# zehreken/fo-rma

Hardware: AMD Instinct MI355X
Metric: Msamples/sec (pixels×spp) at 1920×1080, 256 spp, 8 bounces; 1/2/4/8 GPU (higher is better)
Workload: dtype f32

## Files before the change

fo-rma_amd/csrc/rt_core.h:

```cpp
#pragma once
#include <stdint.h>

#if defined(__HIPCC_RTC__)
#define FR_HD __host__ __device__ __forceinline__
#elif defined(__HIPCC__) || defined(__HIP__)
#include <hip/hip_runtime.h>
#define FR_HD __host__ __device__ __forceinline__
#else
#include <math.h>
#define FR_HD static inline
#endif

namespace fr {

struct V3 {
  float x, y, z;
};

FR_HD V3 mk(float x, float y, float z) { return V3{x, y, z}; }
FR_HD V3 add(V3 a, V3 b) { return V3{a.x + b.x, a.y + b.y, a.z + b.z}; }
FR_HD V3 sub(V3 a, V3 b) { return V3{a.x - b.x, a.y - b.y, a.z - b.z}; }
FR_HD V3 mul(V3 a, V3 b) { return V3{a.x * b.x, a.y * b.y, a.z * b.z}; }
FR_HD V3 scl(float s, V3 a) { return V3{s * a.x, s * a.y, s * a.z}; }
FR_HD V3 divs(V3 a, float s) { return V3{a.x / s, a.y / s, a.z / s}; }
// ... 306 lines not shown
  return s;
}

constexpr float kBoxInvClamp = 0x1p100f;
FR_HD float box_inv_clamp(float inv) { return fmin_num(fmax_num(inv, -kBoxInvClamp), kBoxInvClamp); }
FR_HD bool recip_box_ok(float x) {
  const float ax = __builtin_fabsf(x);
  return (ax >= 0x1p-100f) & (ax < 0x1p126f);
}
FR_HD float fmin3_abs(float a, float b, float c) {
#if defined(__HIP_DEVICE_COMPILE__)
  float r;
  asm("v_min3_f32 %0, |%1|, |%2|, |%3|" : "=v"(r) : "v"(a), "v"(b), "v"(c));
  return r;
#else
  return fminf(fminf(fabsf(a), fabsf(b)), fabsf(c));
#endif
}
FR_HD bool recip_box_ok3(V3 d) {
  const float sum = (__builtin_fabsf(d.x) + __builtin_fabsf(d.y)) + __builtin_fabsf(d.z);
  return (fmin3_abs(d.x, d.y, d.z) >= 0x1p-100f) & (sum < 0x1p126f);
}
#if defined(__HIP__)
__device__ __forceinline__ V3 seg_box_inv(V3 d) {
  V3 inv{recip_nr(d.x), recip_nr(d.y), recip_nr(d.z)};
  if (!recip_box_ok3(d)) {
    inv = V3{1.0f / d.x, 1.0f / d.y, 1.0f / d.z};
    inv = V3{box_inv_clamp(inv.x), box_inv_clamp(inv.y), box_inv_clamp(inv.z)};
  }
  return inv;
}
#endif
FR_HD Slab slab3_box(V3 lo, V3 hi, V3 o, V3 inv, V3 oinv) {
  (void)o;
  return slab3_fused(lo, hi, oinv, inv);
}

FR_HD bool slab_root(const Slab& s, float t_min, float t_max, float& t) {
  t = s.tn > t_min ? s.tn : s.tf;
  return (t > t_min) & (t < t_max) & (s.tn < s.tf);
}

FR_HD float comp(V3 v, int k) { return k == 0 ? v.x : (k == 1 ? v.y : v.z); }

FR_HD V3 axis_normal(int k, float s) {
  return V3{k == 0 ? s : 0.0f, k == 1 ? s : 0.0f, k == 2 ? s : 0.0f};
}

FR_HD V3 slab_normal(const Slab& s, float t, V3 dd) {
#if defined(__HIP_DEVICE_COMPILE__)
  const bool entry = t == s.tn;
  const float mnx = fmin_num(s.t0.x, s.t1.x), mxx = fmax_num(s.t0.x, s.t1.x);
  const float mny = fmin_num(s.t0.y, s.t1.y), mxy = fmax_num(s.t0.y, s.t1.y);
  const bool kx = (entry ? mnx : mxx) == t;
  const bool ky = !kx && (entry ? mny : mxy) == t;
  const bool kz = !kx && !ky;
  const float dk = kx ? dd.x : (ky ? dd.y : dd.z);
  const float sg = ((dk > 0.0f) != entry) ? 1.0f : -1.0f;
  return V3{kx ? sg : 0.0f, ky ? sg : 0.0f, kz ? sg : 0.0f};
#else
  if (t == s.tn) {
    const int k = fmin_num(s.t0.x, s.t1.x) == s.tn ? 0 : (fmin_num(s.t0.y, s.t1.y) == s.tn ? 1 : 2);
    return axis_normal(k, comp(dd, k) > 0.0f ? -1.0f : 1.0f);
  }
  const int k = fmax_num(s.t0.x, s.t1.x) == s.tf ? 0 : (fmax_num(s.t0.y, s.t1.y) == s.tf ? 1 : 2);
  return axis_normal(k, comp(dd, k) > 0.0f ? 1.0f : -1.0f);
#endif
}

FR_HD bool tri_root(V3 v0, V3 e1, V3 e2, V3 o, V3 d, float t_min, float t_max, float& t) {
  const V3 pv = cross(d, e2);
  const float inv_det = 1.0f / dot(e1, pv);
  const V3 s = sub(o, v0);
  const float u = dot(s, pv) * inv_det;
  const V3 qv = cross(s, e1);
  const float v = dot(d, qv) * inv_det;
  t = dot(e2, qv) * inv_det;
  return (u >= 0.0f) & (v >= 0.0f) & (u + v <= 1.0f) & (t > t_min) & (t < t_max);
}

struct ObbFrame {
  V3 dl, inv, ol;
};

FR_HD ObbFrame obb_frame(V3 c, V3 ax, V3 ay, V3 az, V3 o, V3 d) {
  ObbFrame f;
  const V3 oc = sub(o, c);
  f.ol = V3{dot(ax, oc), dot(ay, oc), dot(az, oc)};
  f.dl = V3{dot(ax, d), dot(ay, d), dot(az, d)};
  f.inv = V3{1.0f / f.dl.x, 1.0f / f.dl.y, 1.0f / f.dl.z};
  return f;
}

FR_HD V3 obb_normal(V3 ax, V3 ay, V3 az, const Slab& s, float t, V3 dl) {
  const V3 nl = slab_normal(s, t, dl);
  const float sg = nl.x + nl.y + nl.z;
  const V3 axis = nl.x != 0.0f ? ax : (nl.y != 0.0f ? ay : az);
  return scl(sg, axis);
}

enum ScatterClass : uint32_t { SC_LAMBERT = 0, SC_METAL = 1, SC_DIELECTRIC = 2, SC_LIGHT = 3, SC_NONE = 4 };

FR_HD V3 scatter_lambert(V3 p, V3 n, Rng& r) {
  const V3 target = add(add(p, n), random_in_unit_sphere(r));
  return sub(target, p);
}

FR_HD bool scatter_metal(V3 d, V3 p_unused, V3 n, float fuzz, Rng& r, V3& dir) {
  (void)p_unused;
  const V3 refl = reflect(unit(d), n);
  dir = add(refl, scl(fuzz, random_in_unit_sphere(r)));
  return dot(dir, n) > 0.0f;
}

FR_HD V3 scatter_dielectric(V3 d, V3 n, Rng& r) {
  const float ref_idx = 1.3f;
  const V3 reflected = reflect(d, n);
  V3 outward;
  float ni, cosine;
  const float dn = dot(d, n);
  if (dn > 0.0f) {
    outward = sub(V3{0.0f, 0.0f, 0.0f}, n);
    ni = ref_idx;
    cosine = ref_idx * dot(d, n) / length(d);
  } else {
    outward = n;
    ni = 1.0f / ref_idx;
    cosine = -dot(d, n) / length(d);
  }
  const V3 uv = unit(d);
  const float dt = dot(uv, outward);
  const float disc = 1.0f - ni * ni * (1.0f - dt * dt);
  V3 refracted = V3{0.0f, 0.0f, 0.0f};
  float reflect_prob;
  if (disc > 0.0f) {
    refracted = sub(scl(ni, sub(uv, scl(dt, outward))), scl(sqrtf(disc), outward));
    reflect_prob = schlick(cosine, ref_idx);
  } else {
    reflect_prob = 1.0f;
  }
  return rng_f32(r) < reflect_prob ? reflected : refracted;
}

FR_HD float sky_t(V3 d) {
  const V3 ud = unit(d);
  return 0.5f * (ud.y + 1.0f);
}
FR_HD float sky_t_from(float dy, float dd) { return 0.5f * (dy / sqrtf(dd) + 1.0f); }
FR_HD V3 sky_from_t(float t) { return add(scl(1.0f - t, V3{1.0f, 1.0f, 1.0f}), scl(t, V3{0.5f, 0.7f, 1.0f})); }
FR_HD V3 sky(V3 d) { return sky_from_t(sky_t(d)); }

#if defined(__HIP__)
__device__ __forceinline__ float sky_t_fast_from(float dy, float dd) {
  const bool fast = (dd >= 0x1p-96f) & (dd <= 0x1p126f);
  if (fast) {
#if defined(__HIP_DEVICE_COMPILE__)
    const float s = __builtin_amdgcn_sqrtf(dd);
    const float sdn = __uint_as_float(__float_as_uint(s) - 1u);
    const float sup = __uint_as_float(__float_as_uint(s) + 1u);
    const float rdn = __builtin_fmaf(-sdn, s, dd);
    const float rup = __builtin_fmaf(-sup, s, dd);
    float len = rdn <= 0.0f ? sdn : s;
    len = rup > 0.0f ? sup : len;
    const float q = div_rn(dy, len, recip_nr(len));
    return 0.5f * (q + 1.0f);
#endif
  }
  return sky_t_from(dy, dd);
}
__device__ __forceinline__ float sky_t_fast(V3 d) {
  return sky_t_fast_from(d.y, d.x * d.x + d.y * d.y + d.z * d.z);
}
#endif

FR_HD uint8_t to_u8(float c) {
  const float s = sqrtf(c) * 255.0f;
  if (!(s > 0.0f)) return 0;
  if (s >= 255.0f) return 255;
  return static_cast<uint8_t>(s);
}

FR_HD uint8_t as_u8_trunc(float v) {
  if (!(v > 0.0f)) return 0;
  if (v >= 255.0f) return 255;
  return static_cast<uint8_t>(v);
}

}
```

fo-rma_amd/csrc/trace_kernel.h:

```cpp
#pragma once
#if !defined(__HIPCC_RTC__)
#include <hip/hip_runtime.h>
#include <float.h>
#include <type_traits>
#include "../../include/forma_rt.h"
#include "bvh.h"
#else
#include <type_traits>
#include "forma_rt.h"
#include "bvh.h"
#ifndef FLT_MAX
#define FLT_MAX __FLT_MAX__
#endif
#endif

#ifdef FR_DIAG
__device__ unsigned long long g_fr_diag_lens[2];
__device__ unsigned long long g_fr_diag_rus[2];
#define FR_DIAG_TRY(arr)                                                           \
  do {                                                                             \
    const unsigned long long m_ = __ballot(1);                                     \
    if ((threadIdx.x & 63u) == static_cast<uint32_t>(__ffsll(m_) - 1)) {             \
      atomicAdd(&arr[0], 1ull);                                                    \
      atomicAdd(&arr[1], static_cast<unsigned long long>(__popcll(m_)));           \
// ... 159 lines not shown
    const unsigned long long m_ = __ballot(1);                                       \
    if ((k) < SC_N && lane == static_cast<uint32_t>(__ffsll(m_) - 1)) {            \
      atomicAdd(&sec_cnt[(k) < SC_N ? (k) : 0], 1u);                               \
      atomicAdd(&sec_cnt[SC_N + ((k) < SC_N ? (k) : 0)], lanes_in(m_));            \
    }                                                                                \
  } while (0)
#else
#define SEC(k) do {} while (0)
#endif

extern "C" __device__ bool fr_inverse_ballot(unsigned long long) __asm("llvm.amdgcn.inverse.ballot.i64");
__device__ __forceinline__ bool lane_in(unsigned long long m) { return fr_inverse_ballot(m); }

__device__ __forceinline__ uint32_t lanes_in(unsigned long long m) {
  return static_cast<uint32_t>(__builtin_popcount(static_cast<uint32_t>(m)) +
                               __builtin_popcount(static_cast<uint32_t>(m >> 32)));
}
__device__ __forceinline__ uint32_t lanes_in_once(unsigned long long m) {
  uint32_t c = static_cast<uint32_t>(__builtin_popcountll(m));
#if defined(__HIP_DEVICE_COMPILE__)
  asm("" : "+s"(c));
#endif
  return c;
}
__device__ __forceinline__ uint32_t lanes_set(bool b) { return lanes_in(__builtin_amdgcn_ballot_w64(b)); }

__device__ __forceinline__ uint32_t lds_addr(const uint32_t* p) {
  return static_cast<uint32_t>(reinterpret_cast<uintptr_t>((__attribute__((address_space(3))) const uint32_t*)p));
}
__device__ __forceinline__ __attribute__((address_space(3))) uint32_t& lds_u32_at(uint32_t a) {
  return *reinterpret_cast<__attribute__((address_space(3))) uint32_t*>(static_cast<uintptr_t>(a));
}
__device__ __forceinline__ uint32_t lane_sel(unsigned long long m, uint32_t if_set, uint32_t if_clear) {
#if defined(__HIP_DEVICE_COMPILE__)
  uint32_t r;
  asm("v_cndmask_b32 %0, %1, %2, %3" : "=v"(r) : "v"(if_clear), "v"(if_set), "s"(m));
  return r;
#else
  return if_set;
#endif
}

__device__ __forceinline__ uint32_t slot_tile(const KParams& kp, uint32_t q) {
  uint32_t tile = q >> 6;
#if defined(__HIP_DEVICE_COMPILE__)
  if (kp.flags & KF_LIST) tile = kp.tile_list[__builtin_amdgcn_readfirstlane(tile)];
#endif
  return tile;
}

template <bool LIST = true>
__device__ __forceinline__ bool slot_xy(const KParams& kp, uint32_t q, uint32_t& x, uint32_t& y) {
  const uint32_t tile = LIST ? slot_tile(kp, q) : q >> 6, l = q & 63u;
  const uint32_t ls = fastdiv(tile, kp.row_magic, kp.row_shift);
  const uint32_t tc = tile - ls * kp.tiles_per_row;
  const uint32_t strip = kp.shard_index + ls * kp.shard_count;
  x = tc * 8u + (l & 7u);
  y = strip * kStripRows + (l >> 3);
  return x < kp.W && y < kp.H;
}

__device__ __forceinline__ bool item_xy(const KParams& kp, uint32_t item, uint32_t& bw, uint32_t& q, uint32_t& x,
                                        uint32_t& y) {
  const bool fine = item >= kp.n_coarse;
  const uint32_t tb = (fine ? item - kp.n_coarse : item) >> 6;
  const uint32_t bl = fastdiv(tb, kp.tiles_magic, kp.tiles_shift);
  bw = fine ? (kp.b_fine | kFineKey | (bl << 28)) : kp.b0 + bl;
  q = ((tb - bl * kp.n_tiles) << 6) | (item & 63u);
  return slot_xy(kp, q, x, y);
}

__host__ __device__ __forceinline__ uint32_t stream_key(uint32_t bw) {
  return (bw & kFineKey) ? (kFineKey | ((bw & 0x0FFFFFFFu) * kFineSub + ((bw >> 28) & 3u))) : bw;
}

__device__ __forceinline__ BatchEntry batch_entry(const KParams& kp, uint32_t item) {
  uint32_t bw, q, x, y;
  const bool in_image = item_xy(kp, item, bw, q, x, y);
  const Rng st = rng_seed(kp.seed, y * kp.W + x, stream_key(bw));
  const uint32_t k = (bw >> 28) & 3u;
  const bool fine = (bw & kFineKey) != 0u;
  const uint32_t first = k * kFineSamples;
  const uint32_t left = kp.spp - (bw & 0x0FFFFFFFu) * kBlockSamples;
  const uint32_t span = first + (fine ? kFineSamples : kBlockSamples);
  const uint32_t end = span < left ? span : left;
  const bool ok = in_image && item < kp.n_items;
  BatchEntry e;
  e.s0 = st.s0;
  e.s1 = st.s1;
  e.s2 = st.s2;
  e.s3 = st.s3;
  e.fx = static_cast<float>(x) * 16777216.0f + 8388608.0f;
  e.fy = static_cast<float>(kp.H - y) * 16777216.0f + 8388608.0f;
  const uint64_t slot = static_cast<uint64_t>(item - k * kp.P) * kp.ks;
  e.se = (ok ? (first | (end << 8) | (kNeedJit << 16)) : 0u) | (static_cast<uint32_t>(slot >> 32) << 24);
  e.slot = static_cast<uint32_t>(slot);
  return e;
}

typedef uint32_t u32x4 __attribute__((ext_vector_type(4)));
__device__ __forceinline__ __attribute__((address_space(3))) u32x4& lds_u32x4_at(uint32_t a) {
  return *reinterpret_cast<__attribute__((address_space(3))) u32x4*>(static_cast<uintptr_t>(a));
}
__device__ __forceinline__ void wave_lds_order() {
#if defined(__HIP_DEVICE_COMPILE__)
  __builtin_amdgcn_fence(__ATOMIC_SEQ_CST, "wavefront");
  __builtin_amdgcn_wave_barrier();
#endif
}


template <uint32_t I, uint32_t N, class F>
__device__ __forceinline__ void unroll_below(uint32_t n, F& f) {
  if constexpr (I < N) {
    if (I < n) {
      f(std::integral_constant<uint32_t, I>{});
      unroll_below<I + 1u, N>(n, f);
    }
  }
}

#ifdef FR_JIT_N
constexpr uint32_t kJitRec[FR_JIT_N][16] = {FR_JIT_REC};
template <uint32_t I>
struct JitRec {
  __device__ __forceinline__ float4 operator[](int k) const {
    return make_float4(__builtin_bit_cast(float, kJitRec[I][4 * k]), __builtin_bit_cast(float, kJitRec[I][4 * k + 1]),
                       __builtin_bit_cast(float, kJitRec[I][4 * k + 2]),
                       __builtin_bit_cast(float, kJitRec[I][4 * k + 3]));
  }
};
#endif

template <int KS, bool HAS_PLANE, int KREJ, int MAXD, bool BVH, bool MT, int DEFER, int MAT = 0>
#define FR_OCC_ATTR                                                                                      \
  __attribute__((amdgpu_waves_per_eu(FR_MIN_WAVES ? FR_MIN_WAVES : BVH ? FR_BVH_WAVES                 \
                                                      : DEFER == 2 ? FR_NIB_WAVES                       \
                                                      : (DEFER == 1 && MAT == 1) ? FR_DIFF12_WAVES : 7)))
__global__ __launch_bounds__(kBlock) __attribute__((amdgpu_num_sgpr(FR_NUM_SGPR))) FR_OCC_ATTR void trace_kernel(
    KArgs args) {
  const KScene& sc = args.sc;
  const KParams& kp = args.kp;
  const KWork& kw = args.kw;
  extern __shared__ uint32_t lds[];
  constexpr bool NIB = DEFER == 2;
  constexpr uint32_t STG = stage_samples(BVH, NIB);
  constexpr bool DIFFUSE = MAT == 1;
  constexpr uint32_t WPS = NIB ? 2u : 3u;
  constexpr bool TABLE = has_batch_table(BVH, NIB);
  constexpr uint32_t TABW = TABLE ? kBatchTableBytes / 4u : 0u;
  static_assert(!TABLE || !MT, "a batch-table entry holds no render_mt band offset");
  const bool staged = STG > 1 && (!BVH || NIB || (kp.flags & KF_STAGE) != 0u);
  float* stage = reinterpret_cast<float*>(lds) + TABW + threadIdx.x * (WPS * STG);
  constexpr bool ATT_LDS = DEFER != 0 && !BVH, REC_LDS = NIB && !BVH;
  static_assert(kDeferMaxPrims <= kAttLds && kNibbleMaxPrims <= kRecLds, "LDS staging bounds");
  const uint32_t n_att = ATT_LDS || sc.n <= kAttLds ? sc.n : 0u;
  const uint32_t n_att_st = n_att ? n_att + 1u : 0u;
  const uint32_t n_rec = REC_LDS || sc.n <= kRecLds ? sc.n : 0u;
  float4* att_lds = reinterpret_cast<float4*>(lds + TABW + (staged ? kBlock * WPS * STG : 0u));
  float4* rec_lds = att_lds + n_att_st;
  uint32_t* stack = reinterpret_cast<uint32_t*>(rec_lds + 4u * n_rec);
  uint16_t* hstack = reinterpret_cast<uint16_t*>(stack);
  const uint32_t tid = threadIdx.x;
  const uint32_t lane = tid & 63u;
  static_assert(MAXD == 0 || MAXD == 8, "the u16 stack is one 16-B row per lane");
  static_assert(!DEFER || (MAXD == 8 && !MT && (!BVH || (NIB && DIFFUSE))),
                "deferred unwind: depth <= 8 list kernels, or diffuse BVH kernels with 8-B records");
  uint2* drow = reinterpret_cast<uint2*>(stack) + tid;
  uint8_t* bstack = reinterpret_cast<uint8_t*>(stack);
  uint4* hrow = reinterpret_cast<uint4*>(stack) + tid;
  uint32_t* tstack = stack + (NIB ? 0u : MAXD ? (MAXD * kBlock) / 2u : (kp.max_depth ? kp.max_depth : 1u) * kBlock);
  constexpr uint32_t kLevelB = 4u * kBlock;
  const uint32_t tbase = lds_addr(tstack) + kLevelB;
  if (BVH) tstack[tid] = kBvhEnd;
  const uint32_t ent_shift = n_att ? 4u : 0u;
  const uint32_t unit_ent = sc.n << ent_shift;
  const uint32_t unit2 = unit_ent | (unit_ent << 16);
  if (DEFER == 1)
    *drow = make_uint2(~0u, ~0u);
  else if (!DEFER && MAXD > 0)
    *hrow = make_uint4(unit2, unit2, unit2, unit2);
  for (uint32_t i = tid; i < n_att_st; i += kBlock) {
    const float4 a = sc.att[i];
    att_lds[i] = make_float4(a.x, a.y, a.z, __uint_as_float(i < n_att ? sc.cls[i] : 0u));
  }
  for (uint32_t i = tid; i < 4u * n_rec; i += kBlock) rec_lds[i] = sc.rec[i];
#ifdef FR_DIAG
  __shared__ uint32_t dg[DG_N];
  if (tid < DG_N) dg[tid] = 0;
  const uint32_t gw = blockIdx.x * (kBlock / 64u) + (tid >> 6);
  if (lane == 0 && gw < 65536) {
    g_fr_wave_times[2 * gw] = __builtin_amdgcn_s_memrealtime();
    g_fr_wave_drain[gw] = ~0ull;
  }
#endif
#ifdef FR_SECCNT
  __shared__ uint32_t sec_cnt[2 * SC_N];
  if (tid < 2 * SC_N) sec_cnt[tid] = 0;
#endif
  __syncthreads();


  enum : uint32_t { NEED_NONE = 0, NEED_LENS = 1, NEED_SPHERE = 2, NEED_JIT = 3 };
  static_assert(NEED_JIT == kNeedJit && NEED_NONE == 0u, "a batch-table entry holds the claim's need");
  uint32_t depth = 0;
  uint32_t wnib = ~0u;
  const uint32_t dmask = kp.max_depth ? (0xFu << (4u * (8u - min(kp.max_depth, 8u)))) : 0u;
  auto push = [&](uint32_t pi) {
    if (NIB)
      wnib = (wnib >> 4) | (pi << 28);
    else if (DEFER)
      bstack[tid * 8u + depth] = static_cast<uint8_t>(pi);
    else if (MAXD > 0)
      hstack[tid * MAXD + depth] = static_cast<uint16_t>(pi << ent_shift);
    else
      stack[depth * kBlock + tid] = pi;
  };

  V3 o{0.0f, 0.0f, 0.0f}, d{0.0f, 0.0f, 1.0f};
  V3 sn{0.0f, 0.0f, 0.0f};
  float sfuzz = 0.0f, fx = 0.0f, fy = 0.0f, vofs = 0.0f;
  bool smetal = false;
  uint32_t sbest = 0, s = 0, s_end = 0, nseg = 0, nhit = 0;
  static_assert((kBlockSamples & (kBlockSamples - 1u)) == 0u, "blocks of a power-of-two sample count");
#ifdef FR_DIAG
  uint32_t diag_tb = 0, diag_seg0 = 0;
  uint32_t diag_iter = 0;
#endif
  float* out = kw.samples;
  Rng rng{0u, 0u, 0u, 0u};
  bool active = true, have_ray = false;
  uint32_t need = NEED_NONE;

#ifdef FR_PROF
  uint64_t pf_acc[PF_N] = {0, 0, 0, 0, 0};
  uint64_t pf_t = __builtin_amdgcn_s_memtime();
#endif
  uint32_t q_next = 0, q_end = 0;
  Rng held{0u, 0u, 0u, 0u};
  uint32_t held_xy = 0xFFFFFFFFu, held_b = 0u;
  const uint32_t tab_mine = lds_addr(lds) + tid * kBatchEntryBytes;
  auto seed_entry = [&](const KParams& kq, uint32_t item) {
    const BatchEntry e = batch_entry(kq, item);
    lds_u32x4_at(tab_mine) = u32x4{e.s0, e.s1, e.s2, e.s3};
    lds_u32x4_at(tab_mine + 16u) = u32x4{__float_as_uint(e.fx), __float_as_uint(e.fy), e.se, e.slot};
  };
  {
    const KParams k0 = kernarg_reload(args, [](const auto& a) { return a.kp; });
    q_next = (blockIdx.x * (kBlock / 64u) + (tid >> 6)) * kBatch;
    q_end = q_next + kBatch;
    if constexpr (TABLE) {
      seed_entry(k0, q_next + lane);
      wave_lds_order();
    } else {
      uint32_t bb, qq, xx, yy;
      const bool in_image = item_xy(k0, q_next + lane, bb, qq, xx, yy);
      held = rng_seed(k0.seed, yy * k0.W + xx, stream_key(bb));
      held_xy = in_image ? (xx | (yy << 16)) : 0xFFFFFFFFu;
      held_b = bb;
    }
  }
  while (active) {
    SEC(SC_ITER);
    DIAG_WAVE(DG_ITER);
#ifdef FR_DIAG
    if (lane == 0 && (gw & 63u) == 0 && (gw >> 6) < 1024u && diag_iter < 1024u)
      g_fr_iter_times[(gw >> 6) * 1024u + diag_iter] = __builtin_amdgcn_s_memrealtime();
    ++diag_iter;
#endif
    const unsigned long long m = __builtin_amdgcn_ballot_w64(s == s_end);
    constexpr uint32_t CLAIM_MIN = NIB ? (BVH ? FR_CLAIM_MIN_BVH : FR_CLAIM_MIN_NIB) : FR_CLAIM_MIN;
    if (m && (CLAIM_MIN <= 1 || lanes_in_once(m) >= CLAIM_MIN || m == __ballot(1))) {
      SEC(SC_CLAIM);
      const uint32_t n = static_cast<uint32_t>(__popcll(m));
      const uint32_t r = __builtin_amdgcn_mbcnt_hi(static_cast<uint32_t>(m >> 32),
                                                   __builtin_amdgcn_mbcnt_lo(static_cast<uint32_t>(m), 0u));
      const uint32_t next = __builtin_amdgcn_readfirstlane(q_next);
      const uint32_t avail = __builtin_amdgcn_readfirstlane(q_end) - next;
      if constexpr (TABLE) {
        const bool grab = avail == 0u;
        unsigned long long mc = m;
        uint32_t take = n, start = next;
        if (!grab && n > avail) {
          mc = m & __builtin_amdgcn_ballot_w64(r < avail);
          take = avail;
        }
        if (grab) {
          SEC(SC_GRAB);
          wave_lds_order();
          const int first = __ffsll(static_cast<long long>(m)) - 1;
          uint32_t base = 0;
          if (static_cast<int>(lane) == first) base = atomicAdd(kw.queue, kBatch);
          base = __builtin_amdgcn_readlane(base, first);
          const KParams kg = kernarg_reload(args, [](const auto& a) { return a.kp; });
          base += kg.n_static;
          q_end = base + kBatch;
          seed_entry(kg, base + lane);
          wave_lds_order();
          start = base;
        }
        q_next = start + take;
        const uint32_t item = start + r;
        if (lane_in(mc) && item >= kp.n_items) {
#ifdef FR_DIAG
          if (gw < 65536) {
            const unsigned long long now = __builtin_amdgcn_s_memrealtime();
            if (now < g_fr_wave_drain[gw]) {
              g_fr_wave_drain[gw] = now;
              g_fr_wave_iters[2 * gw] = diag_iter;
            }
          }
#endif
          active = false;
          continue;
        }
        if (lane_in(mc)) {
          SEC(SC_SETUP);
          const uint32_t ea = lds_addr(lds) + (tid & ~63u) * kBatchEntryBytes + (item & (kBatch - 1u)) * kBatchEntryBytes;
          const u32x4 e0 = lds_u32x4_at(ea), e1 = lds_u32x4_at(ea + 16u);
          rng = Rng{e0.x, e0.y, e0.z, e0.w};
          fx = __uint_as_float(e1.x);
          fy = __uint_as_float(e1.y);
          s = e1.z & 0xFFu;
          s_end = (e1.z >> 8) & 0xFFu;
          need = (e1.z >> 16) & 0xFFu;
          uint64_t slot = (static_cast<uint64_t>(e1.z >> 24) << 32) | e1.w;
#if defined(__HIP_DEVICE_COMPILE__)
          asm volatile("" : "+v"(slot));
#endif
          out = kw.samples + WPS * slot;
#ifdef FR_DIAG
          if (s != s_end) {
            diag_tb = item >> 6;
            diag_seg0 = nseg;
          }
#endif
        }
      } else {
        uint32_t base = 0;
        const bool grab = n > avail;
        const int first = __ffsll(static_cast<long long>(m)) - 1;
        int sl = static_cast<int>(((next + r) & (kBatch - 1u)) << 2);
        Rng st{static_cast<uint32_t>(__builtin_amdgcn_ds_bpermute(sl, static_cast<int>(held.s0))),
               static_cast<uint32_t>(__builtin_amdgcn_ds_bpermute(sl, static_cast<int>(held.s1))),
               static_cast<uint32_t>(__builtin_amdgcn_ds_bpermute(sl, static_cast<int>(held.s2))),
               static_cast<uint32_t>(__builtin_amdgcn_ds_bpermute(sl, static_cast<int>(held.s3)))};
        uint32_t xy = static_cast<uint32_t>(__builtin_amdgcn_ds_bpermute(sl, static_cast<int>(held_xy)));
        uint32_t b = static_cast<uint32_t>(__builtin_amdgcn_ds_bpermute(sl, static_cast<int>(held_b)));
        if (grab) {
          SEC(SC_GRAB);
          if (static_cast<int>(lane) == first) base = atomicAdd(kw.queue, kBatch);
          base = __builtin_amdgcn_readlane(base, first);
          const KParams kg = kernarg_reload(args, [](const auto& a) { return a.kp; });
          base += kg.n_static;
          q_end = base + kBatch;
          uint32_t bb, qq, xx, yy;
          const bool in_image = item_xy(kg, base + lane, bb, qq, xx, yy);
          held = rng_seed(kg.seed, yy * kg.W + xx, stream_key(bb));
          held_xy = in_image ? (xx | (yy << 16)) : 0xFFFFFFFFu;
          held_b = bb;
          sl = static_cast<int>(((r - avail) & (kBatch - 1u)) << 2);
          const Rng st2{static_cast<uint32_t>(__builtin_amdgcn_ds_bpermute(sl, static_cast<int>(held.s0))),
                        static_cast<uint32_t>(__builtin_amdgcn_ds_bpermute(sl, static_cast<int>(held.s1))),
                        static_cast<uint32_t>(__builtin_amdgcn_ds_bpermute(sl, static_cast<int>(held.s2))),
                        static_cast<uint32_t>(__builtin_amdgcn_ds_bpermute(sl, static_cast<int>(held.s3)))};
          const uint32_t xy2 = static_cast<uint32_t>(__builtin_amdgcn_ds_bpermute(sl, static_cast<int>(held_xy)));
          const uint32_t b2 = static_cast<uint32_t>(__builtin_amdgcn_ds_bpermute(sl, static_cast<int>(held_b)));
          if (r >= avail) {
            st = st2;
            xy = xy2;
            b = b2;
          }
        }
        q_next = grab ? base + (n - avail) : next + n;
        const uint32_t item = r < avail ? next + r : base + (r - avail);
        if (lane_in(m) && item >= kp.n_items) {
#ifdef FR_DIAG
          if (gw < 65536) {
            const unsigned long long now = __builtin_amdgcn_s_memrealtime();
            if (now < g_fr_wave_drain[gw]) {
              g_fr_wave_drain[gw] = now;
              g_fr_wave_iters[2 * gw] = diag_iter;
            }
          }
#endif
          active = false;
          continue;
        }
        if (lane_in(m)) {
          SEC(SC_SETUP);
          const uint32_t x = xy & 0xFFFFu, y = xy >> 16;
          bool ok = xy != 0xFFFFFFFFu;
          uint32_t yrow = kp.H - y;
          if (MT) {
            const uint32_t k = kp.band_h ? y / kp.band_h : 4u;
            ok = ok && k < 4u;
            yrow = kp.band_h - (y - k * kp.band_h);
            vofs = static_cast<float>(3u - k) * 0.25f;
          }
          if (ok) {
            rng = st;
            const uint32_t k = (b >> 28) & 3u;
            const bool fine = (b & kFineKey) != 0u;
            const uint32_t j0 = k * kFineSamples;
            s = (b & 0x0FFFFFFFu) * kBlockSamples + j0;
            out = kw.samples + WPS * (static_cast<size_t>(item - k * kp.P) * kp.ks);
#ifdef FR_DIAG
            diag_tb = item >> 6;
            diag_seg0 = nseg;
#endif
            s_end = min(s + (fine ? kFineSamples : kBlockSamples), kp.spp);
            fx = static_cast<float>(x) * 16777216.0f + 8388608.0f;
            fy = static_cast<float>(yrow) * 16777216.0f + 8388608.0f;
            need = NEED_JIT;
          }
        }
      }
    }
    PROF_MARK(PF_CLAIM);
    bool ended = false;
    V3 term{0.0f, 0.0f, 0.0f};
    uint32_t tsky;
#if defined(__HIP_DEVICE_COMPILE__)
    asm volatile("" : "=v"(tsky));
#else
    tsky = kDeferAbsorbed;
#endif
    if (need != NEED_NONE) {
      SEC(SC_NEED);
      const unsigned long long msph = __builtin_amdgcn_ballot_w64(need == NEED_SPHERE);
      float pz = 0.0f;
      DIAG_WAVE(DG_LENS_W);
      DIAG_LANE(DG_LENS_L);
      float px = rng_signed_unit_scaled(rng);
      float py = rng_signed_unit_scaled(rng);
      const unsigned long long mjit = __builtin_amdgcn_ballot_w64(need == NEED_JIT);
      float pw = 0.0f;
      if (lane_in(msph | mjit)) pw = rng_signed_unit_scaled(rng);
      if (lane_in(msph)) pz = pw;
      if (lane_in(mjit)) {
        SEC(SC_JIT);
        d.x = div_rn(fx + px, kp.sW, kp.rW);
        d.y = div_rn(fy + py, kp.sH, kp.rH);
        if (MT) d.y = d.y + vofs;
        px = pw;
        py = rng_signed_unit_scaled(rng);
        need = NEED_LENS;
      }
      float dd = px * px + py * py + pz * pz;
      unsigned long long mrej = __builtin_amdgcn_ballot_w64(dd >= kUnitBallScaled);
      while (lanes_in(mrej) > static_cast<uint32_t>(KREJ)) {
        SEC(SC_REJ);
        DIAG_WAVE(DG_LENS_W);
        DIAG_LANE(DG_LENS_L);
        if (lane_in(mrej)) {
          px = rng_signed_unit_scaled(rng);
          py = rng_signed_unit_scaled(rng);
          if (lane_in(msph)) pz = rng_signed_unit_scaled(rng);
          dd = px * px + py * py + pz * pz;
        }
        mrej = __builtin_amdgcn_ballot_w64(dd >= kUnitBallScaled);
      }
      SEC(SC_ACC);
      const unsigned long long macc = ~mrej;
      if (lane_in(macc & ~msph)) {
        SEC(SC_CAM);
        KCam cm = kernarg_reload(args, [](const auto& a) { return a.cam; });
#if defined(__HIP_DEVICE_COMPILE__)
        asm volatile("" : "+s"(cm.dz));
#endif
        const CamLens rd = cam_lens(cm, px, py);
        uint32_t general = (cm.lens_pre & kCamAxial) ^ kCamAxial;
#if defined(__HIP_DEVICE_COMPILE__)
        asm volatile("" : "+s"(general));
#endif
        if (cm.lens_pre & kCamAxial) {
          const CamRay cr = cam_ray_axial(cm, rd, d.x, d.y);
          o = cr.o;
          d = cr.d;
        }
        if (general) {
          const CamRay cr = cam_ray(cm, rd, d.x, d.y);
          o = cr.o;
          d = cr.d;
        }
        if (!NIB) depth = 0;
        have_ray = true;
      }
      if (lane_in(macc & msph)) {
        SEC(SC_SCAT);
        bool ok = true;
        V3 dir;
        if (!DIFFUSE && smetal) {
          const V3 r{px * kSignedUnitScale, py * kSignedUnitScale, pz * kSignedUnitScale};
          dir = add(d, scl(sfuzz, r));
          ok = dot(dir, sn) > 0.0f;
        } else {
          const V3 dr{__builtin_fmaf(px, kSignedUnitScale, d.x), __builtin_fmaf(py, kSignedUnitScale, d.y),
                      __builtin_fmaf(pz, kSignedUnitScale, d.z)};
          dir = sub(dr, o);
        }
        if (ok) {
          if (!(NIB && DIFFUSE)) push(sbest);
          if (!NIB) ++depth;
          d = dir;
          have_ray = true;
        } else {
          ended = true;
          tsky = kDeferAbsorbed;
        }
      }
      if (lane_in(macc)) need = NEED_NONE;
    }
    PROF_MARK(PF_REJ);
    if (have_ray) {
      SEC(SC_HIT);
      ++nseg;
      const V3 inv = seg_box_inv(d);
      const V3 boinv{o.x * inv.x, o.y * inv.y, o.z * inv.z};
      const float a_dd = dot(d, d);
      const SphereSeg ssg = sphere_seg(a_dd);
      float closest = FLT_MAX, t_last = 0.0f;
      int best = -1;
      bool list_walk = !BVH;
      if (BVH) {
        const float ao = fmax3_num(__builtin_fabsf(o.x), __builtin_fabsf(o.y), __builtin_fabsf(o.z));
        const float ad = fmax3_num(__builtin_fabsf(d.x), __builtin_fabsf(d.y), __builtin_fabsf(d.z));
        const float aoi = fmax3_num(__builtin_fabsf(boinv.x), __builtin_fabsf(boinv.y), __builtin_fabsf(boinv.z));
        list_walk = __ballot(!(ao <= sc.reach) | !(ad >= kBvhTinyDir) | !(aoi <= FLT_MAX)) != 0;
      }
      if (BVH && !list_walk) {
        typedef __attribute__((address_space(4))) const uint32_t cu32;
        for (uint32_t sg = 0; sg < sc.n_segs; ++sg) {
          const cu32* sp = (cu32*)(reinterpret_cast<uintptr_t>(sc.segs)) + 4u * __builtin_amdgcn_readfirstlane(sg);
          if (HAS_PLANE && sp[0]) {
            const uint32_t i = sp[3];
            const RecRef r4 = rec_at(sc.rec, i);
            float t = 0.0f;
            const int r = plane_test(xyz(r4[0]), xyz(r4[1]), xyz(r4[2]), o, d, 0.001f, closest, t);
            if (r) t_last = t;
            if (r == 2) {
              closest = t;
              best = static_cast<int>(i);
            }
            continue;
          }
          uint32_t ref = sp[1];
          uint32_t tso = tbase + 4u * tid;
          const V3 invc{__builtin_amdgcn_fmed3f(inv.x, -kBvhInvClamp, kBvhInvClamp),
                        __builtin_amdgcn_fmed3f(inv.y, -kBvhInvClamp, kBvhInvClamp),
                        __builtin_amdgcn_fmed3f(inv.z, -kBvhInvClamp, kBvhInvClamp)};
          const V3 oinv{o.x * invc.x, o.y * invc.y, o.z * invc.z};
          while (ref != kBvhEnd) {
            while (ref < kBvhLeaf) {
              SEC(SC_NODE);
              DIAG_WAVE(DG_NODE_W);
              DIAG_LANE(DG_NODE_L);
#ifdef FR_DIAG
              {
                unsigned long long m_ = __ballot(1);
                uint32_t u_ = 0;
                while (m_ && u_ < 5) {
                  const uint32_t r_ = __builtin_amdgcn_readlane(ref, __ffsll(m_) - 1);
                  m_ &= ~__ballot(ref == r_);
                  ++u_;
                }
                if (u_ == 1) DIAG_WAVE(DG_NCOH_W);
                if (u_ == 2) DIAG_WAVE(DG_NU2_W);
                if (u_ == 3 || u_ == 4) DIAG_WAVE(DG_NU4_W);
                if (depth == 0) DIAG_LANE(DG_NPRIM_L);
              }
#endif
              typedef unsigned long long Mask;
              const uint32_t tdown = tso - kLevelB;
              const uint32_t top = lds_u32_at(tdown);
              uint32_t t_near, t_far;
              Mask t_many, t_both;
              auto node_pick = [&](const Slab& sl, const Slab& sr, const uint32_t cl, const uint32_t cr) {
                const Mask ml = __builtin_amdgcn_ballot_w64(sl.tn <= sl.tf) &
                                __builtin_amdgcn_ballot_w64(sl.tf >= 0.001f) & __builtin_amdgcn_ballot_w64(sl.tn <= closest);
                const Mask mr = __builtin_amdgcn_ballot_w64(sr.tn <= sr.tf) &
                                __builtin_amdgcn_ballot_w64(sr.tf >= 0.001f) & __builtin_amdgcn_ballot_w64(sr.tn <= closest);
                const Mask mgol = ml & (__builtin_amdgcn_ballot_w64(sl.tn <= sr.tn) | ~mr);
                const Mask many = ml | mr;
                const uint32_t cx = cl ^ cr;
                const uint32_t near = cl ^ lane_sel(mgol, 0u, cx);
                t_near = near;
                t_far = near ^ cx;
                t_many = many;
                t_both = ml & mr;
              };
              auto node_step = [&](const float4 na, const float4 nb, const float4 nc, const uint32_t cl,
                                   const uint32_t cr) {
                node_pick(slab3_fused(xyz(na), xyz(nb), oinv, invc),
                          slab3_fused(V3{na.w, nc.x, nc.y}, V3{nb.w, nc.z, nc.w}, oinv, invc), cl, cr);
              };
              const uint32_t ref0 = __builtin_amdgcn_readfirstlane(ref);
              if (__ballot(ref != ref0) == 0) {
                const RecRef nd = rec_at(sc.bvh, ref0);
                const float4 r = nd[3];
                SEC(SC_NODES);
                node_step(nd[0], nd[1], nd[2], __float_as_uint(r.x), __float_as_uint(r.y));
                asm volatile("; bvh node step: scalar");
              } else {
                SEC(SC_NODEV);
                const uint32_t nb0 = ref * 64u;
                const uint4 nr = __builtin_bit_cast(uint4, buf_load4(sc.bvh, nb0 + 48u));
                node_step(buf_load4(sc.bvh, nb0), buf_load4(sc.bvh, nb0 + 16u), buf_load4(sc.bvh, nb0 + 32u), nr.x, nr.y);
                asm volatile("; bvh node step: vector");
              }
              SEC(SC_NODET);
              lds_u32_at(tso) = t_far;
              const uint32_t tpop = lane_sel(t_many, tso, tdown);
              ref = lane_sel(t_many, t_near, top);
              tso = lane_sel(t_both, tso + kLevelB, tpop);
            }
            if (ref == kBvhEnd) break;
            SEC(SC_LEAF);
            DIAG_WAVE(DG_LEAF_W);
            DIAG_LANE(DG_LEAF_L);
            auto leaf_test = [&](const uint32_t i, const auto& r) {
              const float tmax =
// ... 11 lines not shown
              } else if (k == FR_AABB) {
                h = slab_root(slab3_box(xyz(r[0]), xyz(r[1]), o, inv, boinv), 0.001f, tmax, t);
              } else if (k == FR_TRIANGLE) {
                h = tri_root(xyz(r[0]), xyz(r[1]), xyz(r[2]), o, d, 0.001f, tmax, t);
              } else if (k == FR_OBB) {
                const float4 a = r[0], b = r[1], c = r[2], e = r[3];
                const ObbFrame f = obb_frame(xyz(a), xyz(b), xyz(c), xyz(e), o, d);
                h = slab_root(slab3(V3{-a.w, -b.w, -c.w}, V3{a.w, b.w, c.w}, f.ol, f.inv), 0.001f, tmax, t);
              }
              if (h) {
                closest = t;
                best = static_cast<int>(i);
                if (HAS_PLANE) t_last = t;
              }
            };
            const uint32_t first = ref & ((1u << kBvhSlotBits) - 1u);
            const uint32_t cnt = ((ref >> kBvhSlotBits) & 15u) + 1u;
            const uint32_t leaf0 = __builtin_amdgcn_readfirstlane(ref);
            if (__ballot(ref != leaf0) == 0) {
              typedef __attribute__((address_space(4))) const uint32_t cu32l;
              const cu32l* ord = (cu32l*)(reinterpret_cast<uintptr_t>(sc.bvh_order));
              const uint32_t first0 = leaf0 & ((1u << kBvhSlotBits) - 1u);
              const uint32_t cnt0 = ((leaf0 >> kBvhSlotBits) & 15u) + 1u;
              for (uint32_t kk = 0; kk < cnt0; ++kk) {
                SEC(SC_LTESTS);
                leaf_test(ord[first0 + kk], rec_at(sc.lrec, first0 + kk));
              }
              asm volatile("; bvh leaf: scalar");
            } else {
              for (uint32_t kk = 0; kk < cnt; ++kk) {
                SEC(SC_LTESTV);
                const uint32_t slot = first + kk;
                struct LeafRec {
                  const float4* base;
                  uint32_t off;
                  __device__ float4 operator[](uint32_t k) const { return buf_load4(base, off + 16u * k); }
                } const r{sc.lrec, slot * 64u};
                leaf_test(buf_load1(sc.bvh_order, slot * 4u), r);
              }
              asm volatile("; bvh leaf: vector");
            }
            tso -= kLevelB;
            ref = lds_u32_at(tso);
          }
        }
      }
      auto test_rec = [&](auto kind_tag, uint32_t i, const auto& r4) {
        constexpr uint32_t K = decltype(kind_tag)::value;
        float t = 0.0f;
        bool h = false;
        if constexpr (K == FR_AABB) {
          h = slab_root(slab3_box(xyz(r4[0]), xyz(r4[1]), o, inv, boinv), 0.001f, closest, t);
        } else if constexpr (K == FR_SPHERE) {
          const float4 g = r4[0];
          h = sphere_root_fast(xyz(g), g.w, o, d, a_dd, ssg, 0.001f, closest, t);
        } else if constexpr (K == FR_PLANE) {
          const int r = plane_test(xyz(r4[0]), xyz(r4[1]), xyz(r4[2]), o, d, 0.001f, closest, t);
          if (r) t_last = t;
          h = r == 2;
        } else if constexpr (K == FR_TRIANGLE) {
          h = tri_root(xyz(r4[0]), xyz(r4[1]), xyz(r4[2]), o, d, 0.001f, closest, t);
        } else if constexpr (K == FR_OBB) {
          const float4 a = r4[0], b = r4[1], c = r4[2], e = r4[3];
          const ObbFrame f = obb_frame(xyz(a), xyz(b), xyz(c), xyz(e), o, d);
          h = slab_root(slab3(V3{-a.w, -b.w, -c.w}, V3{a.w, b.w, c.w}, f.ol, f.inv), 0.001f, closest, t);
        }
        if (h) {
          closest = t;
          best = static_cast<int>(i);
          if (HAS_PLANE) t_last = t;
        }
#if defined(FR_JIT_N) && defined(__HIP_DEVICE_COMPILE__)
        if constexpr (!std::is_same<typename std::decay<decltype(r4)>::type, RecRef>::value) {
          asm volatile("" : "+v"(best));
          if (HAS_PLANE) asm volatile("" : "+v"(t_last));
        }
#endif
      };
      auto test_one = [&](auto kind_tag, uint32_t i) {
        SEC(SC_LIST);
        test_rec(kind_tag, i, rec_at(sc.rec, i));
      };
      typedef std::integral_constant<uint32_t, FR_AABB> TagAabb;
      typedef std::integral_constant<uint32_t, FR_SPHERE> TagSphere;
#ifdef FR_JIT_N
      if constexpr (!BVH) {
        auto test_j = [&](auto ic) {
          constexpr uint32_t I = decltype(ic)::value;
          constexpr uint32_t K = kJitRec[I][15];
          if constexpr (K == FR_AABB || K == FR_SPHERE || K == FR_PLANE || K == FR_TRIANGLE || K == FR_OBB) {
            test_rec(std::integral_constant<uint32_t, K>{}, I, JitRec<I>{});
          }
        };
        unroll_below<0u, FR_JIT_N>(FR_JIT_N, test_j);
      } else
#endif
      if constexpr (NIB && !BVH && KS != KS_ANY) {
        auto test_k = [&](auto ic) {
          if constexpr (KS == KS_AABB)
            test_one(TagAabb{}, decltype(ic)::value);
          else
            test_one(TagSphere{}, decltype(ic)::value);
        };
        uint32_t n_here = sc.n;
#if defined(__HIP_DEVICE_COMPILE__)
        asm volatile("" : "+s"(n_here));
#endif
        unroll_below<0u, kNibbleMaxPrims>(n_here, test_k);
      } else if constexpr (KS != KS_ANY) {
        for (uint32_t ii = 0; ii < (list_walk ? sc.n : 0u); ++ii) {
          const uint32_t i = __builtin_amdgcn_readfirstlane(ii);
          if constexpr (KS == KS_AABB)
            test_one(TagAabb{}, i);
          else
            test_one(TagSphere{}, i);
        }
      } else {
        typedef __attribute__((address_space(4))) const uint32_t cu32r;
        for (uint32_t rr = 0; rr < (list_walk ? sc.n_runs : 0u); ++rr) {
          const cu32r* rp = (cu32r*)(reinterpret_cast<uintptr_t>(sc.runs)) + 4u * __builtin_amdgcn_readfirstlane(rr);
          const uint32_t k = rp[0], i0 = rp[1], i1 = rp[2];
          if (k == FR_AABB) {
            for (uint32_t i = i0; i < i1; ++i) test_one(TagAabb{}, __builtin_amdgcn_readfirstlane(i));
          } else if (k == FR_SPHERE) {
            for (uint32_t i = i0; i < i1; ++i) test_one(TagSphere{}, __builtin_amdgcn_readfirstlane(i));
          } else if (k == FR_PLANE) {
            for (uint32_t i = i0; i < i1; ++i)
              test_one(std::integral_constant<uint32_t, FR_PLANE>{}, __builtin_amdgcn_readfirstlane(i));
          } else if (k == FR_TRIANGLE) {
            for (uint32_t i = i0; i < i1; ++i)
              test_one(std::integral_constant<uint32_t, FR_TRIANGLE>{}, __builtin_amdgcn_readfirstlane(i));
          } else if (k == FR_OBB) {
            for (uint32_t i = i0; i < i1; ++i)
              test_one(std::integral_constant<uint32_t, FR_OBB>{}, __builtin_amdgcn_readfirstlane(i));
          }
        }
      }
      PROF_MARK(PF_HIT);
      SEC(SC_POSTHIT);
      if (best < 0) {
        SEC(SC_SKY);
        if (DEFER)
          tsky = __float_as_uint(sky_t_fast(d));
        else
          term = sky(d);
        ended = true;
        have_ray = false;
      } else {
        DIAG_WAVE(DG_HIT_W);
        ++nhit;
        ended = true;
        tsky = kDeferAbsorbed;
        have_ray = false;
        if (NIB ? (dmask != 0u && (wnib & dmask) == dmask) : depth < kp.max_depth) {
          SEC(SC_SHADE);
          const V3 pw = add(o, scl(closest, d));
          float4 b0, b1, b2, b3;
          if (REC_LDS || n_rec) {
            const float4* rb = rec_lds + 4 * best;
            b0 = rb[0];
            b1 = rb[1];
            b2 = rb[2];
            b3 = rb[3];
          } else {
            const uint32_t off = 64u * static_cast<uint32_t>(best);
            b0 = buf_load4(sc.rec, off);
            b1 = buf_load4(sc.rec, off + 16u);
            b2 = buf_load4(sc.rec, off + 32u);
            b3 = buf_load4(sc.rec, off + 48u);
          }
          const uint32_t c = (DIFFUSE && KS != KS_ANY) ? static_cast<uint32_t>(SC_LAMBERT)
                             : ATT_LDS || n_att        ? __float_as_uint(att_lds[best].w)
                                                       : buf_load1(sc.cls, 4u * best);
          const uint32_t kb = KS == KS_AABB ? FR_AABB : KS == KS_SPHERE ? FR_SPHERE : __float_as_uint(b3.w);
          V3 n;
          if (kb == FR_AABB) {
            n = slab_normal(slab3_box(xyz(b0), xyz(b1), o, inv, boinv), closest, d);
          } else if (kb == FR_SPHERE) {
            n = divs(sub(pw, xyz(b0)), b0.w);
          } else if (kb == FR_PLANE) {
            n = scl(-1.0f, xyz(b1));
          } else if (kb == FR_TRIANGLE) {
            n = xyz(b3);
            if (c != SC_DIELECTRIC && dot(n, d) > 0.0f) n = scl(-1.0f, n);
          } else {
            const ObbFrame f = obb_frame(xyz(b0), xyz(b1), xyz(b2), xyz(b3), o, d);
            const Slab sl = slab3(V3{-b0.w, -b1.w, -b2.w}, V3{b0.w, b1.w, b2.w}, f.ol, f.inv);
            n = obb_normal(xyz(b1), xyz(b2), xyz(b3), sl, closest, f.dl);
          }
          const V3 p = HAS_PLANE ? add(o, scl(t_last, d)) : pw;
          const V3 din = d;
          o = p;
          d = add(p, n);
          sbest = static_cast<uint32_t>(best);
          smetal = !DIFFUSE && c == SC_METAL;
          ended = c == SC_NONE;
          if (c != SC_NONE && (DIFFUSE || c != SC_DIELECTRIC)) need = NEED_SPHERE;
          if (NIB && DIFFUSE && c != SC_NONE) {
            if (BVH)
              push(buf_load1(sc.acls, 4u * static_cast<uint32_t>(best)));
            else
              push(static_cast<uint32_t>(best));
          }
          if (!DIFFUSE && c == SC_DIELECTRIC) {
            d = scatter_dielectric(din, n, rng);
            push(static_cast<uint32_t>(best));
            if (!NIB) ++depth;
            have_ray = true;
          } else if (smetal) {
            sfuzz = sc.mat[best].w;
            sn = n;
            d = reflect(unit(din), n);
          }
        }
      }
    }
    PROF_MARK(PF_SHADE);
    SEC(SC_POSTSHADE);
    if (ended) {
      SEC(SC_END);
      DIAG_WAVE(DG_END_W);
      DIAG_LANE(DG_END_L);
      V3 col = term;
      if (NIB) {
        col = V3{__uint_as_float(tsky), __uint_as_float(wnib), 0.0f};
        wnib = ~0u;
      } else if (DEFER) {
        const uint2 w = *drow;
        *drow = make_uint2(~0u, ~0u);
        col = V3{__uint_as_float(tsky), __uint_as_float(w.x), __uint_as_float(w.y)};
      } else if (MAXD > 0) {
        const uint4 w = *hrow;
        *hrow = make_uint4(unit2, unit2, unit2, unit2);
        const uint32_t ws[4] = {w.x, w.y, w.z, w.w};
        if (n_att) {
          const char* att_bytes = reinterpret_cast<const char*>(att_lds);
#pragma unroll
          for (int j = MAXD - 1; j >= 0; --j) {
            DIAG_WAVE(DG_UNW_W);
            const uint32_t off = (j & 1) ? (ws[j >> 1] >> 16) : (ws[j >> 1] & 0xFFFFu);
            col = mul(xyz(*reinterpret_cast<const float4*>(att_bytes + off)), col);
          }
        } else {
#pragma unroll
          for (int j = MAXD - 1; j >= 0; --j)
            if (j < static_cast<int>(depth)) col = mul(xyz(sc.att[(ws[j >> 1] >> (16 * (j & 1))) & 0xFFFFu]), col);
        }
      } else {
        const bool zero_term = (__float_as_uint(term.x) | __float_as_uint(term.y) | __float_as_uint(term.z)) == 0u;
        const int udepth = sc.att_nonneg && zero_term ? 0 : static_cast<int>(depth);
        if (n_att) {
          for (int j = udepth - 1; j >= 0; --j) {
            const uint32_t pi = stack[j * kBlock + tid];
            col = mul(xyz(att_lds[pi]), col);
          }
        } else {
          for (int j = udepth - 1; j >= 0; --j) col = mul(xyz(sc.att[stack[j * kBlock + tid]]), col);
        }
      }
      const uint32_t jj = s & (kBlockSamples - 1u);
      if (!staged) {
        out[WPS * jj] = col.x;
        out[WPS * jj + 1] = col.y;
        if (WPS == 3) out[WPS * jj + 2] = col.z;
      } else {
        float* sl = stage + WPS * (jj & (STG - 1u));
        sl[0] = col.x;
        sl[1] = col.y;
        if (WPS == 3) sl[2] = col.z;
        const bool full = (jj & (STG - 1u)) == STG - 1u;
        if (full || s + 1u == s_end) {
          float* dst = out + WPS * (jj & ~(STG - 1u));
          if (full && kp.ks == kBlockSamples) {
            if constexpr ((WPS * STG) % 4u == 0u) {
              const float4* src = reinterpret_cast<const float4*>(stage);
#pragma unroll
              for (uint32_t k = 0; k < WPS * STG / 4u; ++k) {
                reinterpret_cast<float4*>(dst)[k] = src[k];
#if defined(__HIP_DEVICE_COMPILE__)
                if (WPS * STG > 8u) asm volatile("" ::: "memory");
#endif
              }
            } else {
              const float2* src = reinterpret_cast<const float2*>(stage);
#pragma unroll
              for (uint32_t k = 0; k < WPS * STG / 2u; ++k) reinterpret_cast<float2*>(dst)[k] = src[k];
            }
          } else {
            for (uint32_t k = 0; k < WPS * ((jj & (STG - 1u)) + 1u); ++k) dst[k] = stage[k];
          }
        }
      }
#ifdef FR_DIAG
      if (s + 1u == s_end && diag_tb < (1u << 20)) atomicAdd(&g_fr_tb_cost[diag_tb], nseg - diag_seg0);
#endif
      if (++s != s_end) need = NEED_JIT;
    }
    PROF_MARK(PF_END);
    SEC(SC_LATCH);
  }

  unsigned long long a = nseg, b = nhit, sct = 0;
  for (int m = 32; m > 0; m >>= 1) {
    a += __shfl_xor(a, m);
    b += __shfl_xor(b, m);
    sct += __shfl_xor(sct, m);
  }
  if (lane == 0) {
    unsigned long long* wc = kw.wave_counters + 3u * (blockIdx.x * (kBlock / 64u) + (tid >> 6));
    wc[0] = a;
    wc[1] = b;
    wc[2] = sct;
  }
#ifdef FR_SECCNT
  __syncthreads();
  if (tid < SC_N) atomicAdd(&kw.counters[4 + tid], static_cast<unsigned long long>(sec_cnt[tid]));
  if (tid < SC_N) atomicAdd(&kw.counters[32 + tid], static_cast<unsigned long long>(sec_cnt[SC_N + tid]));
#endif
#ifdef FR_PROF
  if (lane == 0)
    for (int k = 0; k < PF_N; ++k) atomicAdd(&kw.counters[20 + k], static_cast<unsigned long long>(pf_acc[k]));
#endif
#ifdef FR_DIAG
  if (lane == 0 && gw < 65536) {
    g_fr_wave_times[2 * gw + 1] = __builtin_amdgcn_s_memrealtime();
    g_fr_wave_iters[2 * gw + 1] = diag_iter;
  }
  __syncthreads();
  if (tid < DG_N) atomicAdd(&kw.counters[4 + tid], static_cast<unsigned long long>(dg[tid]));
#endif
}

}
```

Measured before the change: 40000.

## Make trace loop control wave-uniform with live mask and scalar-friendly branching

Replaces the per-lane active flag with a wave-level live lane mask so the persistent loop exits uniformly, and turns per-lane claim/retire and staging-flush conditions into ballot masks. It also makes the sky-t fast path branchless, forces some values into scalar registers, rewrites the rejection loop as if/do-while, swaps shfl_xor for direct ds_bpermute, and adds an optional compile-time primitive count. The goal is less divergent control flow, fewer exec-mask manipulations and lower register pressure in the hot loop. The cost is more subtle mask logic with risk of correctness issues, and the branchless sky path always computes both variants.

New measurement: 40010 (median of 2 runs). No clear change (+0.0%).

```diff
diff --git a/fo-rma_amd/csrc/rt_core.h b/fo-rma_amd/csrc/rt_core.h
--- a/fo-rma_amd/csrc/rt_core.h
+++ b/fo-rma_amd/csrc/rt_core.h
@@ -482,21 +482,22 @@
 
 #if defined(__HIP__)
 __device__ __forceinline__ float sky_t_fast_from(float dy, float dd) {
+#if defined(__HIP_DEVICE_COMPILE__)
   const bool fast = (dd >= 0x1p-96f) & (dd <= 0x1p126f);
-  if (fast) {
-#if defined(__HIP_DEVICE_COMPILE__)
-    const float s = __builtin_amdgcn_sqrtf(dd);
-    const float sdn = __uint_as_float(__float_as_uint(s) - 1u);
-    const float sup = __uint_as_float(__float_as_uint(s) + 1u);
-    const float rdn = __builtin_fmaf(-sdn, s, dd);
-    const float rup = __builtin_fmaf(-sup, s, dd);
-    float len = rdn <= 0.0f ? sdn : s;
-    len = rup > 0.0f ? sup : len;
-    const float q = div_rn(dy, len, recip_nr(len));
-    return 0.5f * (q + 1.0f);
-#endif
-  }
+  const float s = __builtin_amdgcn_sqrtf(dd);
+  const float sdn = __uint_as_float(__float_as_uint(s) - 1u);
+  const float sup = __uint_as_float(__float_as_uint(s) + 1u);
+  const float rdn = __builtin_fmaf(-sdn, s, dd);
+  const float rup = __builtin_fmaf(-sup, s, dd);
+  float len = rdn <= 0.0f ? sdn : s;
+  len = rup > 0.0f ? sup : len;
+  const float q = div_rn(dy, len, recip_nr(len));
+  float t = 0.5f * (q + 1.0f);
+  if (!fast) t = sky_t_from(dy, dd);
+  return t;
+#else
   return sky_t_from(dy, dd);
+#endif
 }
 __device__ __forceinline__ float sky_t_fast(V3 d) {
   return sky_t_fast_from(d.y, d.x * d.x + d.y * d.y + d.z * d.z);
diff --git a/fo-rma_amd/csrc/trace_kernel.h b/fo-rma_amd/csrc/trace_kernel.h
--- a/fo-rma_amd/csrc/trace_kernel.h
+++ b/fo-rma_amd/csrc/trace_kernel.h
@@ -335,11 +335,17 @@
   static_assert(!TABLE || !MT, "a batch-table entry holds no render_mt band offset");
   const bool staged = STG > 1 && (!BVH || NIB || (kp.flags & KF_STAGE) != 0u);
   float* stage = reinterpret_cast<float*>(lds) + TABW + threadIdx.x * (WPS * STG);
+  const unsigned long long wide_ok = __builtin_amdgcn_ballot_w64(kp.ks == kBlockSamples);
   constexpr bool ATT_LDS = DEFER != 0 && !BVH, REC_LDS = NIB && !BVH;
   static_assert(kDeferMaxPrims <= kAttLds && kNibbleMaxPrims <= kRecLds, "LDS staging bounds");
-  const uint32_t n_att = ATT_LDS || sc.n <= kAttLds ? sc.n : 0u;
+#ifdef FR_JIT_N
+  const uint32_t scn = BVH ? sc.n : FR_JIT_N;
+#else
+  const uint32_t scn = sc.n;
+#endif
+  const uint32_t n_att = ATT_LDS || scn <= kAttLds ? scn : 0u;
   const uint32_t n_att_st = n_att ? n_att + 1u : 0u;
-  const uint32_t n_rec = REC_LDS || sc.n <= kRecLds ? sc.n : 0u;
+  const uint32_t n_rec = REC_LDS || scn <= kRecLds ? scn : 0u;
   float4* att_lds = reinterpret_cast<float4*>(lds + TABW + (staged ? kBlock * WPS * STG : 0u));
   float4* rec_lds = att_lds + n_att_st;
   uint32_t* stack = reinterpret_cast<uint32_t*>(rec_lds + 4u * n_rec);
@@ -357,7 +363,7 @@
   const uint32_t tbase = lds_addr(tstack) + kLevelB;
   if (BVH) tstack[tid] = kBvhEnd;
   const uint32_t ent_shift = n_att ? 4u : 0u;
-  const uint32_t unit_ent = sc.n << ent_shift;
+  const uint32_t unit_ent = scn << ent_shift;
   const uint32_t unit2 = unit_ent | (unit_ent << 16);
   if (DEFER == 1)
     *drow = make_uint2(~0u, ~0u);
@@ -389,6 +395,7 @@
   uint32_t depth = 0;
   uint32_t wnib = ~0u;
   const uint32_t dmask = kp.max_depth ? (0xFu << (4u * (8u - min(kp.max_depth, 8u)))) : 0u;
+  const uint32_t dfree = kp.max_depth ? dmask : 1u;
   auto push = [&](uint32_t pi) {
     if (NIB)
       wnib = (wnib >> 4) | (pi << 28);
@@ -412,7 +419,8 @@
 #endif
   float* out = kw.samples;
   Rng rng{0u, 0u, 0u, 0u};
-  bool active = true, have_ray = false;
+  bool have_ray = false;
+  unsigned long long live = ~0ull;
   uint32_t need = NEED_NONE;
 
 #ifdef FR_PROF
@@ -430,7 +438,7 @@
   };
   {
     const KParams k0 = kernarg_reload(args, [](const auto& a) { return a.kp; });
-    q_next = (blockIdx.x * (kBlock / 64u) + (tid >> 6)) * kBatch;
+    q_next = __builtin_amdgcn_readfirstlane((blockIdx.x * (kBlock / 64u) + (tid >> 6)) * kBatch);
     q_end = q_next + kBatch;
     if constexpr (TABLE) {
       seed_entry(k0, q_next + lane);
@@ -443,7 +451,7 @@
       held_b = bb;
     }
   }
-  while (active) {
+  do {
     SEC(SC_ITER);
     DIAG_WAVE(DG_ITER);
 #ifdef FR_DIAG
@@ -451,11 +459,15 @@
       g_fr_iter_times[(gw >> 6) * 1024u + diag_iter] = __builtin_amdgcn_s_memrealtime();
     ++diag_iter;
 #endif
-    const unsigned long long m = __builtin_amdgcn_ballot_w64(s == s_end);
+    const unsigned long long m = __builtin_amdgcn_ballot_w64(s == s_end) & live;
     constexpr uint32_t CLAIM_MIN = NIB ? (BVH ? FR_CLAIM_MIN_BVH : FR_CLAIM_MIN_NIB) : FR_CLAIM_MIN;
-    if (m && (CLAIM_MIN <= 1 || lanes_in_once(m) >= CLAIM_MIN || m == __ballot(1))) {
+    const uint32_t n = lanes_in_once(m);
+    uint32_t claim_at = (CLAIM_MIN > 1 && m != live) ? CLAIM_MIN : 1u;
+#if defined(__HIP_DEVICE_COMPILE__)
+    asm("" : "+s"(claim_at));
+#endif
+    if (n >= claim_at) {
       SEC(SC_CLAIM);
-      const uint32_t n = static_cast<uint32_t>(__popcll(m));
       const uint32_t r = __builtin_amdgcn_mbcnt_hi(static_cast<uint32_t>(m >> 32),
                                                    __builtin_amdgcn_mbcnt_lo(static_cast<uint32_t>(m), 0u));
       const uint32_t next = __builtin_amdgcn_readfirstlane(q_next);
@@ -484,20 +496,18 @@
         }
         q_next = start + take;
         const uint32_t item = start + r;
-        if (lane_in(mc) && item >= kp.n_items) {
+        const unsigned long long mret = mc & __builtin_amdgcn_ballot_w64(item >= kp.n_items);
 #ifdef FR_DIAG
-          if (gw < 65536) {
-            const unsigned long long now = __builtin_amdgcn_s_memrealtime();
-            if (now < g_fr_wave_drain[gw]) {
-              g_fr_wave_drain[gw] = now;
-              g_fr_wave_iters[2 * gw] = diag_iter;
-            }
-          }
-#endif
-          active = false;
-          continue;
-        }
-        if (lane_in(mc)) {
+        if (lane_in(mret) && gw < 65536) {
+          const unsigned long long now = __builtin_amdgcn_s_memrealtime();
+          if (now < g_fr_wave_drain[gw]) {
+            g_fr_wave_drain[gw] = now;
+            g_fr_wave_iters[2 * gw] = diag_iter;
+          }
+        }
+#endif
+        live &= ~mret;
+        if (lane_in(mc & ~mret)) {
           SEC(SC_SETUP);
           const uint32_t ea = lds_addr(lds) + (tid & ~63u) * kBatchEntryBytes + (item & (kBatch - 1u)) * kBatchEntryBytes;
           const u32x4 e0 = lds_u32x4_at(ea), e1 = lds_u32x4_at(ea + 16u);
@@ -509,7 +519,7 @@
           need = (e1.z >> 16) & 0xFFu;
           uint64_t slot = (static_cast<uint64_t>(e1.z >> 24) << 32) | e1.w;
 #if defined(__HIP_DEVICE_COMPILE__)
-          asm volatile("" : "+v"(slot));
+          asm volatile("" : "+v"(slot), "+v"(rng.s0));
 #endif
           out = kw.samples + WPS * slot;
 #ifdef FR_DIAG
@@ -557,20 +567,18 @@
         }
         q_next = grab ? base + (n - avail) : next + n;
         const uint32_t item = r < avail ? next + r : base + (r - avail);
-        if (lane_in(m) && item >= kp.n_items) {
+        const unsigned long long mret = m & __builtin_amdgcn_ballot_w64(item >= kp.n_items);
 #ifdef FR_DIAG
-          if (gw < 65536) {
-            const unsigned long long now = __builtin_amdgcn_s_memrealtime();
-            if (now < g_fr_wave_drain[gw]) {
-              g_fr_wave_drain[gw] = now;
-              g_fr_wave_iters[2 * gw] = diag_iter;
-            }
-          }
-#endif
-          active = false;
-          continue;
-        }
-        if (lane_in(m)) {
+        if (lane_in(mret) && gw < 65536) {
+          const unsigned long long now = __builtin_amdgcn_s_memrealtime();
+          if (now < g_fr_wave_drain[gw]) {
+            g_fr_wave_drain[gw] = now;
+            g_fr_wave_iters[2 * gw] = diag_iter;
+          }
+        }
+#endif
+        live &= ~mret;
+        if (lane_in(m & ~mret)) {
           SEC(SC_SETUP);
           const uint32_t x = xy & 0xFFFFu, y = xy >> 16;
           bool ok = xy != 0xFFFFFFFFu;
@@ -632,7 +640,7 @@
       }
       float dd = px * px + py * py + pz * pz;
       unsigned long long mrej = __builtin_amdgcn_ballot_w64(dd >= kUnitBallScaled);
-      while (lanes_in(mrej) > static_cast<uint32_t>(KREJ)) {
+      if (lanes_in_once(mrej) > static_cast<uint32_t>(KREJ)) do {
         SEC(SC_REJ);
         DIAG_WAVE(DG_LENS_W);
         DIAG_LANE(DG_LENS_L);
@@ -643,14 +651,14 @@
           dd = px * px + py * py + pz * pz;
         }
         mrej = __builtin_amdgcn_ballot_w64(dd >= kUnitBallScaled);
-      }
+      } while (lanes_in_once(mrej) > static_cast<uint32_t>(KREJ));
       SEC(SC_ACC);
       const unsigned long long macc = ~mrej;
       if (lane_in(macc & ~msph)) {
         SEC(SC_CAM);
         KCam cm = kernarg_reload(args, [](const auto& a) { return a.cam; });
 #if defined(__HIP_DEVICE_COMPILE__)
-        asm volatile("" : "+s"(cm.dz));
+        asm volatile("" : "+s"(cm.dz), "+s"(cm.px));
 #endif
         const CamLens rd = cam_lens(cm, px, py);
         uint32_t general = (cm.lens_pre & kCamAxial) ^ kCamAxial;
@@ -968,7 +976,7 @@
         ended = true;
         tsky = kDeferAbsorbed;
         have_ray = false;
-        if (NIB ? (dmask != 0u && (wnib & dmask) == dmask) : depth < kp.max_depth) {
+        if (NIB ? (wnib & dmask) == dfree : depth < kp.max_depth) {
           SEC(SC_SHADE);
           const V3 pw = add(o, scl(closest, d));
           float4 b0, b1, b2, b3;
@@ -1084,10 +1092,12 @@
         sl[0] = col.x;
         sl[1] = col.y;
         if (WPS == 3) sl[2] = col.z;
-        const bool full = (jj & (STG - 1u)) == STG - 1u;
-        if (full || s + 1u == s_end) {
-          float* dst = out + WPS * (jj & ~(STG - 1u));
-          if (full && kp.ks == kBlockSamples) {
+        const unsigned long long mfull = __builtin_amdgcn_ballot_w64((jj & (STG - 1u)) == STG - 1u);
+        const unsigned long long mlast = __builtin_amdgcn_ballot_w64(s + 1u == s_end);
+        const unsigned long long mwide = mfull & wide_ok;
+        float* dst = out + WPS * (jj & ~(STG - 1u));
+        {
+          if (lane_in(mwide)) {
             if constexpr ((WPS * STG) % 4u == 0u) {
               const float4* src = reinterpret_cast<const float4*>(stage);
 #pragma unroll
@@ -1102,7 +1112,8 @@
 #pragma unroll
               for (uint32_t k = 0; k < WPS * STG / 2u; ++k) reinterpret_cast<float2*>(dst)[k] = src[k];
             }
-          } else {
+          }
+          if (lane_in((mfull | mlast) & ~mwide)) {
             for (uint32_t k = 0; k < WPS * ((jj & (STG - 1u)) + 1u); ++k) dst[k] = stage[k];
           }
         }
@@ -1114,13 +1125,19 @@
     }
     PROF_MARK(PF_END);
     SEC(SC_LATCH);
-  }
+  } while (live);
 
   unsigned long long a = nseg, b = nhit, sct = 0;
-  for (int m = 32; m > 0; m >>= 1) {
-    a += __shfl_xor(a, m);
-    b += __shfl_xor(b, m);
-    sct += __shfl_xor(sct, m);
+  auto from_lane = [](int byte_addr, unsigned long long v) {
+    const uint32_t lo = static_cast<uint32_t>(__builtin_amdgcn_ds_bpermute(byte_addr, static_cast<int>(v)));
+    const uint32_t hi = static_cast<uint32_t>(__builtin_amdgcn_ds_bpermute(byte_addr, static_cast<int>(v >> 32)));
+    return (static_cast<unsigned long long>(hi) << 32) | lo;
+  };
+  for (uint32_t m = 32; m > 0; m >>= 1) {
+    const int partner = static_cast<int>((lane ^ m) << 2);
+    a += from_lane(partner, a);
+    b += from_lane(partner, b);
+    sct += from_lane(partner, sct);
   }
   if (lane == 0) {
     unsigned long long* wc = kw.wave_counters + 3u * (blockIdx.x * (kBlock / 64u) + (tid >> 6));
```
